# FofanovLab/mtsv_tools

Hardware: AMD Instinct MI355X
Metric: reads/sec (whole node), 150bp reads vs MG-index (higher is better)
Workload: dtype u32/i16

## Files before the change

mtsv_tools_amd/csrc/batch.hip:

```cpp
#include <atomic>
#include <chrono>
#include <cmath>
#include <condition_variable>
#include <exception>
#include <mutex>
#include <thread>
#include <cstdio>
#include <cstdlib>
#include <cstring>
#include <stdexcept>
#include <vector>

#include "../../include/mtsv_amd.h"
#include "batch.hpp"
#include "kernels.hpp"

namespace mtsv {

namespace {
template <class F>
void parallel_ranges(uint64_t n, F f) {
    static const int max_nt = [] {
        const char* e = getenv("MTSV_COPY_THREADS");
        return e ? std::max(1, std::min(16, atoi(e))) : 4;
// ... 209 lines not shown
    sw_ms_acc = 0;
    sweep_ms_acc = diag_ms_acc = bound_ms_acc = edit_ms_acc = 0;
    sw_passed_acc = 0;
    n_hits_total = 0;
    HIP_CHECK(hipMemsetAsync(d_counters, 0, kCounters * sizeof(uint64_t), stream));
    HIP_CHECK(hipEventRecord(ev[8], stream));
}

void Batch::finish_lane() {
    HIP_CHECK(hipEventRecord(ev[9], stream));
    launch_publish(stream, d_counters, h_counters, kCounters);
    HIP_CHECK(hipStreamSynchronize(stream));
    HIP_CHECK(hipEventElapsedTime(&stage_acc[7], ev[8], ev[9]));
    if (getenv("MTSV_TRACE")) fprintf(stderr, "[lane] last pass: %llu strands of 13..64 seed hits (or more than 4 candidates) to k_coalesce_mid, %llu heavier ones\n",
                                      (unsigned long long)(h_counters[15] & 0xffffffffull), (unsigned long long)(h_counters[1] >> 32));
    stats.sw_cell_pairs = h_counters[14];
    stats.sw_prefilter_ms = sw_ms_acc;
    stats.sw_sweep_ms = sweep_ms_acc;
    stats.sw_diag_ms = diag_ms_acc;
    stats.sw_bound_ms = bound_ms_acc;
    stats.edit_ms = edit_ms_acc;
    stats.myers_columns = h_counters[19];
    stats.n_sw_bound_refuted = h_counters[20];
    stats.n_sw_passed = sw_passed_acc + h_counters[21];
    stats.lf_steps = h_counters[2];
    stats.n_candidates = h_counters[3];
    stats.n_verified = h_counters[4];
    stats.window_bytes = h_counters[5];
}

// ... 179 lines not shown
            dev_alloc(&d_seed_pre, want, &dummy);
            seed_cap = want;
        }
        const bool myers_pass = !tiled && pass_max_len <= 253 && (verify_mode == 1 || (sw_pairs && hit_cap < 0x80000000ull));
        const uint32_t plane_words = myers_pass ? myers_words(pass_max_len) : 0;
        if ((uint64_t)nr * 3 * plane_words > plane_cap) {
            (void)hipFree(d_planes);
            d_planes = nullptr;
            const uint64_t want = std::max<uint64_t>(nr, ws_reads) * 3 * plane_words;
            uint64_t dummy = 0;
            dev_alloc(&d_planes, want, &dummy);
            plane_cap = want;
        }
        HIP_CHECK(hipEventRecord(ev[0], stream));
        const uint32_t listed_cap = (uint32_t)std::min<uint64_t>(slots, std::max<uint64_t>(4096, (uint64_t)((double)slots * listed_share)));
        launch_search(stream, v, sb, so, (uint32_t)r0, nr, max_ns, K, G, d_seed_lo, d_seed_cnt, d_seed_pre, (uint32_t*)(d_counters + 22), listed_cap);
        HIP_CHECK(hipEventRecord(ev[1], stream));
        if (max_ns)
            launch_thin(stream, sb, so, (uint32_t)r0, nr, p.edit_rate, p.min_seed, max_ns, K, G, p.max_hits, p.tune_max_hits, d_seed_cnt,
                        d_seed_pre, d_strand_hits, d_strand_nseeds, myers_pass ? d_planes : nullptr, plane_words);
        else {
            HIP_CHECK(hipMemsetAsync(d_strand_hits, 0, (uint64_t)nstr * 4, stream));
            HIP_CHECK(hipMemsetAsync(d_strand_nseeds, 0, (uint64_t)nstr * 4, stream));
        }
        launch_scan(stream, d_strand_hits, nstr, d_tile_sums, d_counters + 0, d_strand_off);
        launch_publish(stream, d_counters, h_counters, 1);
        launch_publish(stream, d_counters + 22, h_counters + 22, 1);
        HIP_CHECK(hipEventRecord(ev[2], stream));
        HIP_CHECK(hipStreamSynchronize(stream));
        {
            const uint64_t n_listed = h_counters[22] & 0xffffffffull;
// ... 792 lines not shown
```

mtsv_tools_amd/csrc/batch.hpp:

```cpp
#pragma once
#include <memory>
#include <mutex>
#include <vector>

#include "../../include/mtsv_amd.h"
#include "host_pack.hpp"
#include "dev_index.hpp"
#include "kernels.hpp"

namespace mtsv {

struct Batch {
    mtsv_index* ix;
    DeviceIndex* di;
    hipStream_t stream = nullptr, copy_stream2 = nullptr;
    mtsv_hit* h_hits_stage = nullptr;
    uint64_t h_hits_cap = 0, staged_hits = 0, last_total_hits = 0;
    bool staged_valid = false;
    struct Arena {
        uint8_t* d_bases = nullptr;
        uint8_t* d_packed = nullptr;
        uint32_t* d_off = nullptr;
        uint64_t cap_bases = 0, cap_reads = 0;
    };
// ... 35 lines not shown
    uint64_t *d_hit_key = nullptr, *d_cand_tmp = nullptr;
    uint4 *d_cand = nullptr, *d_out = nullptr;
    uint32_t *d_cand_next = nullptr, *d_cand_status = nullptr, *d_heavy_list = nullptr;
    DevHit* d_hits = nullptr;
    uint2* d_strip = nullptr;
    uint64_t strip_cap = 0;
    uint32_t* d_planes = nullptr;
    uint64_t plane_cap = 0;
    uint64_t* h_counters = nullptr;
    hipEvent_t ev[15];
    float sw_ms_acc = 0, sweep_ms_acc = 0, diag_ms_acc = 0, bound_ms_acc = 0, edit_ms_acc = 0;
    uint64_t sw_passed_acc = 0;

    std::vector<uint32_t> h_read_off;
    uint32_t max_len = 0;
    static constexpr int kCounters = 24;
    double listed_share = 0.125;
    bool sw_diag = true;
    bool sw_top = true;
    bool sw_bound = true;
    bool sw_fused = true;
    bool sw_prepass = true;
    bool sw_pairs = true;
    int verify_mode = 0;
    uint64_t n_reads = 0;
    uint64_t n_hits_total = 0;
    mtsv_batch_stats stats{};
    float stage_acc[MTSV_N_STAGES] = {0};

    Batch(mtsv_index* ix, DeviceIndex* di, uint64_t max_reads, uint64_t max_bases, uint64_t hit_cap, Batch* parent = nullptr, int lanes = 0);
    ~Batch();
// ... 50 lines not shown
```

mtsv_tools_amd/csrc/dev_index.hip:

```cpp
#include <algorithm>
#include <cstdio>
#include <cstdlib>
#include <cstring>
#include <stdexcept>
#include <thread>
#include <vector>

#include "dev_index.hpp"

namespace mtsv {

void throw_hip(hipError_t e, const char* what, const char* file, int line) {
    throw std::runtime_error(std::string("device: ") + hipGetErrorString(e) + " at " + what + " (" + file + ":" +
                             std::to_string(line) + ")");
}

DeviceIndex::~DeviceIndex() {
    if (device < 0) return;
    (void)hipSetDevice(device);
    (void)hipFree(d_blocks);
    (void)hipFree(d_sa_sample);
    (void)hipFree(d_sa_full);
    (void)hipFree(d_text);
    (void)hipFree(d_bin_end);
    (void)hipFree(d_bins);
    (void)hipFree(d_bin_lut);
    (void)hipFree(d_kmer);
}

namespace {

inline uint32_t sym_code(uint8_t c) {
    switch (c) {
    case 'A': return kCodeA;
    case 'C': return kCodeC;
    case 'G': return kCodeG;
    case 'T': return kCodeT;
    case 'N': return kCodeN;
    case '$': return kCodeSentinel;
    default: return 7;
    }
}
// ... 255 lines not shown
        uint64_t entries = 1ull << (2 * k);
        uint2 *ta = nullptr, *tb = nullptr;
        if (k == 17) {
            if (hipMalloc((void**)&ta, entries * 8) != hipSuccess || hipMalloc((void**)&tb, entries / 4 * 8) != hipSuccess) {
                (void)hipGetLastError();
                if (ta) (void)hipFree(ta);
                ta = tb = nullptr;
                k = 16;
                entries = 1ull << 32;
            }
        }
        if (!ta) {
            HIP_CHECK(hipMalloc((void**)&ta, entries * 8));
            HIP_CHECK(hipMalloc((void**)&tb, std::max<uint64_t>(entries / 4, 4) * 8));
        }
        uint2* cur = (k % 2 == 1) ? ta : tb;
        uint2* oth = (k % 2 == 1) ? tb : ta;
        hipLaunchKernelGGL(k_kmer_level1, dim3(1), dim3(64), 0, 0, v, cur);
        for (uint32_t lvl = 2; lvl <= k; lvl++) {
            const uint64_t total = 1ull << (2 * lvl);
            hipLaunchKernelGGL(k_kmer_level, dim3((uint32_t)std::min<uint64_t>((total + 255) / 256, 1u << 22)), dim3(256), 0, 0, v, cur, oth,
                               2 * (lvl - 1));
            std::swap(cur, oth);
        }
        HIP_CHECK(hipGetLastError());
        HIP_CHECK(hipDeviceSynchronize());
        HIP_CHECK(hipFree(tb));
        di->d_kmer = ta;
        di->bytes += entries * 8;
        v.kmer_tab = di->d_kmer;
        v.kmer_k = k;
        const char* kp = getenv("MTSV_KMER_POS");
        if (v.sa_full && !(kp && atoi(kp) == 0)) {
            unsigned long long* d_n = nullptr;
            HIP_CHECK(hipMalloc((void**)&d_n, sizeof(unsigned long long)));
            HIP_CHECK(hipMemset(d_n, 0, sizeof(unsigned long long)));
            hipEvent_t t0, t1;
            HIP_CHECK(hipEventCreate(&t0));
            HIP_CHECK(hipEventCreate(&t1));
            HIP_CHECK(hipEventRecord(t0, 0));
            hipLaunchKernelGGL(k_kmer_tag, dim3((uint32_t)std::min<uint64_t>((entries + 255) / 256, 1u << 16)), dim3(256), 0, 0, v,
                               di->d_kmer, entries, d_n);
            HIP_CHECK(hipGetLastError());
            HIP_CHECK(hipEventRecord(t1, 0));
            unsigned long long n_tagged = 0;
            HIP_CHECK(hipMemcpy(&n_tagged, d_n, sizeof(n_tagged), hipMemcpyDeviceToHost));
// ... 22 lines not shown
```

mtsv_tools_amd/csrc/dev_index.hpp:

```cpp
#pragma once
#include <map>
#include <memory>
#include <mutex>
#include <string>

#include "dev_layout.hpp"
#include "mgindex.hpp"

namespace mtsv {

[[noreturn]] void throw_hip(hipError_t e, const char* what, const char* file, int line);
#define HIP_CHECK(expr)                                              \
    do {                                                             \
        hipError_t _e = (expr);                                      \
        if (_e != hipSuccess) ::mtsv::throw_hip(_e, #expr, __FILE__, __LINE__); \
    } while (0)

struct DeviceIndex {
    int device = -1;
    RankBlock* d_blocks = nullptr;
    uint32_t* d_sa_sample = nullptr;
    uint32_t* d_sa_full = nullptr;
    uint8_t* d_text = nullptr;
    uint32_t* d_bin_end = nullptr;
    DevBin* d_bins = nullptr;
    uint32_t* d_bin_lut = nullptr;
    uint2* d_kmer = nullptr;
    DevIndexView view{};
    uint64_t bytes = 0;
    uint32_t flags = 0;
    float accel_build_ms = 0.f;

    DeviceIndex() = default;
    DeviceIndex(const DeviceIndex&) = delete;
    DeviceIndex& operator=(const DeviceIndex&) = delete;
    ~DeviceIndex();
};

std::unique_ptr<DeviceIndex> upload_index(const HostIndex& hx, int device, uint32_t flags);

}

// ... 11 lines not shown
```

mtsv_tools_amd/csrc/dev_layout.hpp:

```cpp
#pragma once
#include <hip/hip_runtime.h>

#include <cstdint>

namespace mtsv {

constexpr uint32_t kCodeA = 0, kCodeC = 1, kCodeG = 2, kCodeT = 3, kCodeN = 4, kCodeSentinel = 5;
constexpr uint32_t kBlockRows = 128;
constexpr uint32_t kBlockShift = 7;

struct alignas(64) RankBlock {
    uint32_t cnt[4];
    uint64_t p0[2];
    uint64_t p1[2];
    uint64_t p2[2];
};
static_assert(sizeof(RankBlock) == 64, "rank block must be one 64-byte line");

struct DevBin {
    uint32_t start, end, tax_id, gi;
};

struct DevIndexView {
    const RankBlock* blocks;
// ... 10 lines not shown
    const DevBin* bins;
    uint32_t n_bins;
    const uint32_t* bin_lut;
    uint32_t bin_lut_shift;
    const uint2* kmer_tab;
    uint32_t kmer_k;
};

constexpr uint32_t kKmerTag = 0xFFFFFF00u;
__host__ __device__ inline bool kmer_tagged(uint2 e) { return (e.y & kKmerTag) == kKmerTag; }
__host__ __device__ inline uint32_t kmer_tag_c1(uint2 e) { return e.y & 7u; }
__host__ __device__ inline uint32_t kmer_tag_c2(uint2 e) { return (e.y >> 3) & 7u; }
__host__ __device__ inline uint2 kmer_tag_entry(uint32_t p, uint32_t c1, uint32_t c2) {
    return make_uint2(p, kKmerTag | c1 | (c2 << 3));
}

constexpr uint32_t kSeedAtPos = 0xFFFFFFFFu;

__host__ __device__ inline uint32_t base_code(uint8_t b) {
    switch (b) {
    case 'A': case 'a': return kCodeA;
    case 'C': case 'c': return kCodeC;
    case 'G': case 'g': return kCodeG;
    case 'T': case 't': return kCodeT;
    default: return kCodeN;
    }
}
__host__ __device__ inline uint32_t comp_code(uint32_t c) { return c < 4 ? 3 - c : c; }

#ifdef __HIPCC__
// ... 57 lines not shown
```

mtsv_tools_amd/csrc/k_coalesce.hip:

```cpp
#include "kernels_common.hpp"

namespace mtsv {

namespace {

__device__ inline uint64_t wave_bitonic_sort(uint64_t key) {
    const uint32_t lane = lane_id();
    for (uint32_t k = 2; k <= kWave; k <<= 1)
        for (uint32_t j = k >> 1; j > 0; j >>= 1) {
            uint64_t other = __shfl_xor(key, j);
            bool up = (lane & k) == 0;
            bool lower = (lane & j) == 0;
            key = (lower == up) ? min(key, other) : max(key, other);
        }
    return key;
}

__device__ inline uint32_t find_bin(const DevIndexView& ix, uint32_t site) {
    const uint32_t k = site >> ix.bin_lut_shift;
    uint32_t lo = ix.bin_lut[k], hi = ix.bin_lut[k + 1];
    while (lo < hi) {
        uint32_t mid = (lo + hi) >> 1;
        if (ix.bin_end[mid] <= site)
            lo = mid + 1;
        else
            hi = mid;
    }
    return lo;
}

__device__ inline bool candidate_window(uint32_t site, uint32_t q, const DevBin& bin, uint32_t L, uint32_t ED,
                                        uint32_t* ws, uint32_t* we) {
    uint32_t start_offset = q + ED;
// ... 92 lines not shown
    uint32_t maxc;
    const uint32_t* strand_off;
    const uint32_t* strand_nseeds;
    const uint32_t* hit_ref;
    const uint32_t* hit_q;
    uint64_t* hit_key;
    uint64_t* cand_tmp;
    uint4* cand;
    uint32_t* cand_next;
    uint32_t* cand_status;
    uint32_t* strand_ncand;
    uint32_t* worklist;
    uint32_t* wl_count;
    unsigned long long* n_cand_total;
};

template <bool BLK>
__device__ void coalesce_big(const DevIndexView& ix, const HeavyArgs& a, uint32_t rs, KeyMem<BLK> km, uint32_t* sh_nc) {
    const uint32_t lane = lane_id();
    const uint32_t tid = km.tid(), nt = km.nthreads();
    const bool walker = !BLK || threadIdx.x < kWave;
    const uint32_t o = a.strand_off[rs];
    const uint32_t nh = a.strand_off[rs + 1] - o;
    const uint32_t ns_raw = a.strand_nseeds[rs];
    const bool hopeless = (ns_raw & kHopeless) != 0;
    const StrandGeom g = strand_geom(a.read_off, a.r0 + (rs >> 1), ns_raw);
    for (uint32_t i = tid; i < nh; i += nt) km.st(i, ((uint64_t)a.hit_ref[o + i] << 32) | a.hit_q[o + i]);
    km.sync();
    big_sort(km, nh);
    uint32_t nc = 0;
    uint64_t* ct = a.cand_tmp + 2ull * o;
    if (walker) {
        Walk w{false, 0, 0, 0, 0};
        for (uint32_t base = 0; base < nh; base += kWave) {
            uint32_t cntv = min((uint32_t)kWave, nh - base);
            uint32_t b = 0, ws = 0, we = 0;
            bool ok = false;
            if (lane < cntv) {
                uint64_t key = km.ld(base + lane);
                uint32_t site = (uint32_t)(key >> 32), q = (uint32_t)key;
                b = min(find_bin(ix, site), ix.n_bins - 1);
                DevBin bin = ix.bins[b];
                ok = candidate_window(site, q, bin, g.L, g.ED, &ws, &we);
            }
            for (uint32_t i = 0; i < cntv; i++) {
                uint32_t wsi = __builtin_amdgcn_readlane(ws, i), wei = __builtin_amdgcn_readlane(we, i);
                uint32_t bi = __builtin_amdgcn_readlane(b, i);
                bool oki = __builtin_amdgcn_readlane((uint32_t)ok, i) != 0;
                bool merge = w.have && oki && bi == w.b && ((w.s <= wsi && wsi < w.e) || (w.s < wei && wei <= w.e));
                if (merge) {
                    w.s = min(w.s, wsi);
                    w.e = max(w.e, wei);
                    w.n++;
                } else {
                    if (w.have && w.n >= g.min_seeds) {
                        if (lane == 0) {
                            gstore(ct + 2ull * nc, ((uint64_t)w.e << 32) | w.s);
                            gstore(ct + 2ull * nc + 1, ((uint64_t)w.n << 32) | w.b);
// ... 21 lines not shown
        unsigned long long wsum = 0;
        for (uint32_t i = tid; i < nc; i += nt) {
            const uint64_t se = gload(ct + 2ull * i);
            wsum += (uint32_t)(se >> 32) - (uint32_t)se;
        }
        for (int d = 32; d > 0; d >>= 1) wsum += __shfl_down(wsum, d);
        if (lane == 0 && wsum) atomicAdd(a.n_cand_total + 2, wsum);
        if (tid == 0) {
            a.strand_ncand[rs] = 0;
            if (nc) {
                atomicAdd(a.n_cand_total, (unsigned long long)nc);
                atomicAdd(a.n_cand_total + 1, (unsigned long long)nc);
            }
        }
        km.sync();
        return;
    }
    for (uint32_t i = tid; i < nc; i += nt) {
        uint32_t n_i = (uint32_t)(gload(ct + 2ull * i + 1) >> 32);
        km.st(i, ((uint64_t)(0xffffffffu - n_i) << 32) | i);
    }
    km.sync();
    big_sort(km, nc);
    for (uint32_t base = 0; base < nc; base += nt) {
        uint32_t i = base + tid;
        uint64_t taxkey = 0;
        if (i < nc) {
            uint32_t src = (uint32_t)km.ld(i);
            uint64_t se = gload(ct + 2ull * src), bn = gload(ct + 2ull * src + 1);
            a.cand[o + i] = make_uint4((uint32_t)se, (uint32_t)(se >> 32), (uint32_t)bn, rs);
            a.cand_status[o + i] = 0;
// ... 21 lines not shown
            emit = (p == 0 || (kp >> 32) != (k0 >> 32)) && rk < a.maxc && !hopeless;
        }
        unsigned long long em = __ballot(emit);
        if (em) {
            uint32_t b2 = 0;
            if (lane == 0) b2 = atomicAdd(a.wl_count, (uint32_t)__popcll(em));
            b2 = __builtin_amdgcn_readfirstlane(b2);
            if (emit) a.worklist[b2 + __popcll(em & ((1ull << lane) - 1))] = o + rk;
        }
    }
    if (tid == 0) {
        a.strand_ncand[rs] = hopeless ? 0 : nc;
        if (nc) atomicAdd(a.n_cand_total, (unsigned long long)nc);
    }
    km.sync();
}

template <uint32_t KEYS>
__global__ __launch_bounds__(256) void k_coalesce_heavy(DevIndexView ix, HeavyArgs a, const uint32_t* __restrict__ heavy_list,
                                                        uint32_t list_len, const uint32_t* __restrict__ heavy_count) {
    __shared__ uint64_t lk[KEYS];
    __shared__ uint32_t sh_nc;
    const uint32_t n_heavy = *heavy_count;
    for (uint32_t h = blockIdx.x; h < n_heavy; h += gridDim.x) {
        const uint32_t rs = heavy_list[list_len - 1 - h];
        const uint32_t nh = a.strand_off[rs + 1] - a.strand_off[rs];
        if (KEYS == kHeavyKeysSmall ? nh > kHeavyKeysSmall : nh <= kHeavyKeysSmall) continue;
        if (nh <= KEYS) {
            coalesce_big<true>(ix, a, rs, KeyMem<true>{lk}, &sh_nc);
        } else {
            if (threadIdx.x < kWave) coalesce_big<false>(ix, a, rs, KeyMem<false>{a.hit_key + a.strand_off[rs]}, nullptr);
            __syncthreads();
        }
    }
}


struct CoalesceArgs {
    const uint32_t* read_off;
    uint32_t r0, n_strands;
    uint32_t maxc;
    const uint32_t* strand_off;
    const uint32_t* strand_nseeds;
    const uint32_t* hit_ref;
    const uint32_t* hit_q;
    uint4* cand;
    uint32_t* cand_next;
    uint32_t* cand_status;
// ... 423 lines not shown
    a.maxc = rank_bound(max_candidates);
    a.strand_off = strand_off;
    a.strand_nseeds = strand_nseeds;
    a.hit_ref = hit_ref;
    a.hit_q = hit_q;
    a.hit_key = hit_key;
    a.cand_tmp = cand_tmp;
    a.cand = cand;
    a.cand_next = cand_next;
    a.cand_status = cand_status;
    a.strand_ncand = strand_ncand;
    a.worklist = worklist;
    a.wl_count = wl_count;
    a.n_cand_total = n_cand_total;
    const dim3 hgrid(std::min<uint32_t>(std::max<uint32_t>(n_strands / 64, 1), 2048));
    hipLaunchKernelGGL(k_coalesce_heavy<kHeavyKeysSmall>, hgrid, dim3(256), 0, s, ix, a, heavy_list, n_strands, heavy_count);
    hipLaunchKernelGGL(k_coalesce_heavy<kHeavyKeys>, dim3(std::min<uint32_t>(hgrid.x, 512)), dim3(256), 0, s, ix, a, heavy_list, n_strands, heavy_count);
}

namespace {
__global__ __launch_bounds__(256) void k_max_window(uint32_t n_strands, const uint32_t* __restrict__ strand_off,
                                                    const uint32_t* __restrict__ strand_ncand, const uint4* __restrict__ cand,
                                                    unsigned long long* __restrict__ out) {
    const uint32_t rs = blockIdx.x * blockDim.x + threadIdx.x;
    uint32_t m = 0;
    if (rs < n_strands) {
        const uint32_t o = strand_off[rs], nc = strand_ncand[rs];
        for (uint32_t i = 0; i < nc; i++) {
            const uint4 c = cand[o + i];
            m = max(m, c.y - c.x);
        }
    }
// ... 12 lines not shown
```

mtsv_tools_amd/csrc/k_seed.hip:

```cpp
#include "kernels_common.hpp"

namespace mtsv {

namespace {

__device__ inline uint32_t fast_code(uint32_t ch);
__global__ __launch_bounds__(256) void k_normalise(const uint8_t* src, uint8_t* dst, uint64_t lo, uint64_t hi) {
    const uint64_t i = (lo & ~15ull) + ((uint64_t)blockIdx.x * blockDim.x + threadIdx.x) * 16;
    if (i >= hi) return;
    if (i < lo || i + 16 > hi) {
        const uint64_t a = i < lo ? lo : i, b = i + 16 > hi ? hi : i + 16;
        for (uint64_t q = a; q < b; q++) dst[q] = (uint8_t)fast_code(src[q]);
        return;
    }
    uint4 v = *reinterpret_cast<const uint4*>(src + i);
    uint32_t w[4] = {v.x, v.y, v.z, v.w};
#pragma unroll
    for (int k = 0; k < 4; k++) {
        uint32_t o = 0;
#pragma unroll
        for (int q = 0; q < 4; q++) o |= fast_code((w[k] >> (8 * q)) & 0xffu) << (8 * q);
        w[k] = o;
    }
    *reinterpret_cast<uint4*>(dst + i) = make_uint4(w[0], w[1], w[2], w[3]);
// ... 19 lines not shown
    *reinterpret_cast<uint4*>(dst + i) = make_uint4(w[0], w[1], w[2], w[3]);
}

__device__ inline uint32_t fast_code(uint32_t ch) {
    uint32_t uc = ch & 0xDFu;
    uint32_t x = (uc >> 1) & 3u;
    uint32_t c = x ^ (x >> 1);
    bool acgt = uc == 'A' || uc == 'C' || uc == 'G' || uc == 'T';
    return acgt ? c : kCodeN;
}

constexpr uint32_t kMaxPackedSeed = 32;

__device__ inline void search_slot(const DevIndexView& ix, const uint8_t* __restrict__ bases, const uint32_t* __restrict__ read_off,
                                   uint32_t r0, uint32_t max_ns, uint32_t K, uint32_t G, uint64_t slot,
                                   uint32_t* __restrict__ seed_lo, uint32_t* __restrict__ seed_cnt) {

    uint32_t j = (uint32_t)(slot % max_ns);
    uint64_t rs = slot / max_ns;
    uint32_t strand = (uint32_t)(rs & 1);
    uint32_t r = r0 + (uint32_t)(rs >> 1);
    uint32_t b0 = read_off[r], L = read_off[r + 1] - b0;
    uint32_t ns = n_seeds_of(L, K, G);
    uint32_t lo = 0, hi = 0;
    bool at_pos = false;
    if (j < ns) {
        const uint8_t* read = bases + b0;
        uint32_t off = j * G;
        uint64_t c_lo = 0, c_hi = 0;
        const bool packed = K <= kMaxPackedSeed;
        const uint32_t s0 = b0 + (strand ? L - off - K : off);
// ... 76 lines not shown
            }
            if (acgt) {
                uint2 iv = ix.kmer_tab[idx];
                lo = iv.x;
                hi = iv.y;
                i = (int)K - 1 - (int)ix.kmer_k;
                if (kmer_tagged(iv)) {
                    const uint32_t p = iv.x, m = (uint32_t)(i + 1);
                    bool match = p >= m;
                    for (uint32_t t = 0; match && t < m; t++) match = sym(t) == ix.text[p - m + t];
                    at_pos = match;
                    lo = match ? p - m : 0;
                    hi = 0;
                    i = -1;
                }
            }
        }
        for (; i >= 0 && lo < hi; i--) {
            uint32_t a = sym((uint32_t)i);
            uint32_t bl = lo >> kBlockShift, bh = hi >> kBlockShift;
            LoadedBlock B0 = load_block(ix.blocks, bl);
            uint32_t nlo = less_of(ix, a) + block_rank(B0, a, bl, lo & (kBlockRows - 1), ix.sentinel_row);
            uint32_t nhi;
            if (bh == bl) {
                nhi = less_of(ix, a) + block_rank(B0, a, bh, hi & (kBlockRows - 1), ix.sentinel_row);
            } else {
                LoadedBlock B1 = load_block(ix.blocks, bh);
                nhi = less_of(ix, a) + block_rank(B1, a, bh, hi & (kBlockRows - 1), ix.sentinel_row);
            }
            lo = nlo;
            hi = nhi;
        }
        if (!at_pos && lo >= hi) lo = hi = 0;
    }
    seed_lo[slot] = lo;
    seed_cnt[slot] = at_pos ? kSeedAtPos : hi - lo;
}

__global__ __launch_bounds__(256) void k_search(DevIndexView ix, const uint8_t* __restrict__ bases,
                                                const uint32_t* __restrict__ read_off, uint32_t r0, uint32_t n_reads,
                                                uint32_t max_ns, uint32_t K, uint32_t G,
                                                uint32_t* __restrict__ seed_lo, uint32_t* __restrict__ seed_cnt) {
    uint64_t slot = (uint64_t)blockIdx.x * blockDim.x + threadIdx.x;
    uint64_t total = (uint64_t)n_reads * 2 * max_ns;
    if (slot >= total) return;
    search_slot(ix, bases, read_off, r0, max_ns, K, G, slot, seed_lo, seed_cnt);
}

template <int KK, bool FRONT_TEXT>
__device__ inline bool fast_slot(const DevIndexView& ix, const uint8_t* __restrict__ bases, const uint32_t* __restrict__ read_off,
                                 uint32_t r0, uint32_t total, uint32_t max_ns, uint32_t K, uint32_t G, uint32_t slot,
                                 uint32_t* __restrict__ seed_lo, uint32_t* __restrict__ seed_cnt) {
    const bool in_range = slot < total;
    const uint32_t rs = in_range ? slot / max_ns : 0, j = in_range ? slot - rs * max_ns : 0;
    const uint32_t strand = rs & 1, r = r0 + (rs >> 1);
    const uint32_t b0 = read_off[r], L = read_off[r + 1] - b0;
    const bool live = in_range && j < n_seeds_of(L, K, G);
    uint32_t lo = 0, hi = 0;
    bool slow = false, at_pos = false;
    if (live) {
        const uint32_t off = j * G;
// ... 148 lines not shown
    if (lane < n_slow) tail_q[at + lane] = slow_q[lane];
    __syncthreads();
    const uint32_t nt = tail_n;
    if (nt) {
        __shared__ uint32_t tail_base;
        if (threadIdx.x == 0) tail_base = atomicAdd(slow_count, nt);
        __syncthreads();
        if (threadIdx.x < nt) slow_list[tail_base + threadIdx.x] = tail_q[threadIdx.x];
    }
}

__global__ __launch_bounds__(256) void k_search_listed(DevIndexView ix, const uint8_t* __restrict__ bases,
                                                       const uint32_t* __restrict__ read_off, uint32_t r0, uint32_t max_ns, uint32_t K,
                                                       uint32_t G, const uint32_t* __restrict__ slow_list,
                                                       const uint32_t* __restrict__ slow_count, uint32_t* __restrict__ seed_lo,
                                                       uint32_t* __restrict__ seed_cnt) {
    const uint32_t i = blockIdx.x * blockDim.x + threadIdx.x;
    if (i >= *slow_count) return;
    search_slot(ix, bases, read_off, r0, max_ns, K, G, slow_list[i], seed_lo, seed_cnt);
}


__global__ __launch_bounds__(256) void k_thin(const uint8_t* __restrict__ bases, const uint32_t* __restrict__ read_off,
                                              uint32_t r0, uint32_t n_reads, double edit_rate, double min_seed,
                                              uint32_t max_ns, uint32_t K, uint32_t G, uint64_t max_hits,
                                              uint64_t tune_max_hits, uint32_t* __restrict__ seed_cnt,
                                              uint32_t* __restrict__ seed_pre, uint32_t* __restrict__ strand_hits,
                                              uint32_t* __restrict__ strand_nseeds, uint32_t* __restrict__ planes,
                                              uint32_t plane_words) {
    uint32_t rs = blockIdx.x * blockDim.x + threadIdx.x;
    if (rs >= n_reads * 2) return;
    uint32_t r = r0 + (rs >> 1);
    const uint32_t b0 = read_off[r];
    uint32_t L = read_off[r + 1] - b0;
// ... 290 lines not shown
}

void launch_normalise(hipStream_t s, const uint8_t* src, uint8_t* dst, uint64_t begin, uint64_t end) {
    if (end <= begin) return;
    const uint64_t n = end - (begin & ~15ull);
    hipLaunchKernelGGL(k_normalise, dim3(cdiv((n + 15) / 16, 256)), dim3(256), 0, s, src, dst, begin, end);
}
void launch_unpack(hipStream_t s, const uint8_t* packed, uint8_t* dst, uint64_t lo, uint64_t hi) {
    if (hi <= lo) return;
    const uint64_t groups = ((hi + 15) >> 4) - (lo >> 4);
    hipLaunchKernelGGL(k_unpack, dim3((uint32_t)cdiv(groups, 256)), dim3(256), 0, s, packed, dst, lo, hi);
}

void launch_search(hipStream_t s, const DevIndexView& ix, const uint8_t* bases, const uint32_t* read_off, uint32_t r0,
                   uint32_t n_reads, uint32_t max_ns, uint32_t K, uint32_t G, uint32_t* seed_lo, uint32_t* seed_cnt,
                   uint32_t* slow_list, uint32_t* slow_count, uint32_t listed_cap) {
    (void)hipMemsetAsync(slow_count, 0, sizeof(uint32_t), s);
    uint64_t total = (uint64_t)n_reads * 2 * max_ns;
    if (!total) return;
    const bool fast = ix.kmer_tab && total < 0xffffffffull && K >= 16 && K <= 24 && ix.kmer_k >= 12 && ix.kmer_k <= 17 &&
                      K >= ix.kmer_k && K - std::min<uint32_t>(ix.kmer_k, 16) <= 8 && !getenv("MTSV_SEARCH_GENERIC");
    if (!fast) {
        hipLaunchKernelGGL(k_search, dim3(cdiv(total, 256)), dim3(256), 0, s, ix, bases, read_off, r0, n_reads, max_ns, K, G,
                           seed_lo, seed_cnt);
        return;
    }
    const dim3 grid(std::min<uint32_t>(cdiv(total, 256), 256 * 16));
#define FAST_CASE(KKV)                                                                                                  \
    if (K - KKV > 2)                                                                                                    \
        hipLaunchKernelGGL((k_search_fast<KKV, true>), grid, dim3(256), 0, s, ix, bases, read_off, r0, (uint32_t)total, max_ns, K, G, \
                           seed_lo, seed_cnt, slow_list, slow_count);                                                   \
    else                                                                                                                \
        hipLaunchKernelGGL((k_search_fast<KKV, false>), grid, dim3(256), 0, s, ix, bases, read_off, r0, (uint32_t)total, max_ns, K, G, \
                           seed_lo, seed_cnt, slow_list, slow_count)
    switch (ix.kmer_k) {
    case 12: FAST_CASE(12); break;
    case 13: FAST_CASE(13); break;
    case 14: FAST_CASE(14); break;
    case 15: FAST_CASE(15); break;
    case 17: FAST_CASE(17); break;
    default: FAST_CASE(16); break;
    }
#undef FAST_CASE
    hipLaunchKernelGGL(k_search_listed, dim3(cdiv(std::max<uint32_t>(listed_cap, 1), 256)), dim3(256), 0, s, ix, bases, read_off, r0, max_ns, K, G,
                       slow_list, slow_count, seed_lo, seed_cnt);
}

void launch_thin(hipStream_t s, const uint8_t* bases, const uint32_t* read_off, uint32_t r0, uint32_t n_reads, double edit_rate,
                 double min_seed, uint32_t max_ns, uint32_t K, uint32_t G, uint64_t max_hits, uint64_t tune, uint32_t* seed_cnt, uint32_t* seed_pre,
                 uint32_t* strand_hits, uint32_t* strand_nseeds, uint32_t* planes, uint32_t plane_words) {
    hipLaunchKernelGGL(k_thin, dim3(cdiv((uint64_t)n_reads * 2, 256)), dim3(256), 0, s, bases, read_off, r0, n_reads, edit_rate,
                       min_seed, max_ns, K, G, max_hits, tune, seed_cnt, seed_pre, strand_hits, strand_nseeds, planes, plane_words);
}

void launch_scan(hipStream_t s, const uint32_t* in, uint32_t n, uint64_t* tile_sums, uint64_t* total, uint32_t* out) {
    uint32_t tiles = cdiv(n ? n : 1, kScanTile);
    hipLaunchKernelGGL(k_scan_tile_sums, dim3(tiles), dim3(kScanThreads), 0, s, in, n, tile_sums);
    hipLaunchKernelGGL(k_scan_sums, dim3(1), dim3(1024), 0, s, tile_sums, tiles, total);
    hipLaunchKernelGGL(k_scan_apply, dim3(tiles), dim3(kScanThreads), 0, s, in, n, tile_sums, total, out);
}
// ... 21 lines not shown
```

mtsv_tools_amd/csrc/kernels.hpp:

```cpp
#pragma once
#include <algorithm>

#include "dev_layout.hpp"

namespace mtsv {

struct DevHit {
    uint64_t read;
    uint32_t tax_id;
    uint32_t gi;
    uint32_t edit;
    uint8_t strand;
    uint8_t pad[3];
    uint64_t offset;
};
static_assert(sizeof(DevHit) == 32, "DevHit must match mtsv_hit");

constexpr uint32_t kCtrVerified = 4, kCtrWindowBytes = 5, kCtrSwCursor = 8, kCtrPassCount = 9, kCtrSwCellPairs = 14;

struct EvalArgs {
    const uint8_t* bases;
    const uint32_t* read_off;
    uint32_t r0;
    double edit_rate;
    int64_t max_candidates;
    const uint32_t* strand_off;
    const uint4* cand;
    const uint32_t* cand_next;
    uint32_t* cand_status;
    const uint32_t* worklist;
    const uint32_t* wl_count;
    uint32_t* wl_cursor;
    uint32_t wl_reverse = 0;
// ... 16 lines not shown
    uint32_t plane_words = 0;
    uint32_t maxc = 0xffffffffu;
    uint32_t claim_shift = 0;
};

inline uint32_t myers_words(uint32_t max_len) { return std::min(std::max((max_len + 31) / 32, 2u), 8u); }

constexpr uint32_t kMaxRegisterReadLen = 256;
constexpr uint32_t kMaxReadLen = 32767;

void launch_publish(hipStream_t s, const uint64_t* src, uint64_t* dst_host, uint32_t n);
void launch_normalise(hipStream_t s, const uint8_t* src, uint8_t* dst, uint64_t begin, uint64_t end);
void launch_unpack(hipStream_t s, const uint8_t* packed, uint8_t* dst, uint64_t lo, uint64_t hi);
void launch_search(hipStream_t s, const DevIndexView& ix, const uint8_t* bases, const uint32_t* read_off, uint32_t r0,
                   uint32_t n_reads, uint32_t max_ns, uint32_t K, uint32_t G, uint32_t* seed_lo, uint32_t* seed_cnt,
                   uint32_t* slow_list, uint32_t* slow_count, uint32_t listed_cap);
void launch_thin(hipStream_t s, const uint8_t* bases, const uint32_t* read_off, uint32_t r0, uint32_t n_reads, double edit_rate,
                 double min_seed, uint32_t max_ns, uint32_t K, uint32_t G, uint64_t max_hits, uint64_t tune, uint32_t* seed_cnt, uint32_t* seed_pre,
                 uint32_t* strand_hits, uint32_t* strand_nseeds, uint32_t* planes, uint32_t plane_words);
void launch_scan(hipStream_t s, const uint32_t* in, uint32_t n, uint64_t* tile_sums, uint64_t* total, uint32_t* out);
uint32_t scan_tiles(uint32_t n);
void launch_expand(hipStream_t s, const DevIndexView& ix, uint32_t n_strands, uint32_t max_ns, uint32_t G,
                   const uint32_t* seed_lo, const uint32_t* seed_cnt, const uint32_t* seed_pre, const uint32_t* strand_off,
                   uint32_t* hit_row, uint32_t* hit_ref, uint32_t* hit_q);
void launch_locate(hipStream_t s, const DevIndexView& ix, uint32_t total_hits_host, const uint32_t* total_hits_dev,
                   const uint32_t* hit_row, uint32_t* hit_ref, unsigned long long* lf_steps);
void launch_coalesce(hipStream_t s, const DevIndexView& ix, const uint32_t* read_off, uint32_t r0, uint32_t n_strands,
                     int64_t max_candidates, const uint32_t* strand_off,
                     const uint32_t* strand_nseeds, const uint32_t* hit_ref, const uint32_t* hit_q, uint64_t* hit_key,
                     uint64_t* cand_tmp, uint4* cand, uint32_t* cand_next, uint32_t* cand_status,
                     uint32_t* strand_ncand, uint32_t* worklist, uint32_t* heavy_list, uint64_t* counters);
// ... 19 lines not shown
```

Before: 396.5 million.

## Parallelize heavy-strand coalescing by bin runs and keep k-mer prefix levels for seeding

The heavy coalesce kernel for strands with up to the small key count now computes candidate windows for all hits across the whole block and merges each run of equal bins in parallel, one thread per run start. A block prefix sum then compacts the kept candidates, and blocks pull strands through an atomic ticket counter instead of a fixed stride. If any run exceeds a length cap, the kernel falls back to the serial wavefront walk, reusing the windows it already computed. Separately, the index builder keeps every intermediate k-mer table level up to 12, so the generic and listed seed-search paths can start backward search from a short-prefix interval when the full k-mer lookup does not apply. This costs extra device memory and shared memory, which may lower occupancy of the heavy kernel.

After: 413.5 million, median of 6. 1.04x the previous value.

```diff
diff --git a/mtsv_tools_amd/csrc/batch.hip b/mtsv_tools_amd/csrc/batch.hip
--- a/mtsv_tools_amd/csrc/batch.hip
+++ b/mtsv_tools_amd/csrc/batch.hip
@@ -247,6 +247,8 @@
     HIP_CHECK(hipEventElapsedTime(&stage_acc[7], ev[8], ev[9]));
     if (getenv("MTSV_TRACE")) fprintf(stderr, "[lane] last pass: %llu strands of 13..64 seed hits (or more than 4 candidates) to k_coalesce_mid, %llu heavier ones\n",
                                       (unsigned long long)(h_counters[15] & 0xffffffffull), (unsigned long long)(h_counters[1] >> 32));
+    if (getenv("MTSV_TRACE")) fprintf(stderr, "[lane] k_coalesce_heavy: %llu strands walked by runs, %llu by the wavefront walk (a run too long)\n",
+                                      (unsigned long long)(h_counters[kCtrHeavyWalk] & 0xffffffffull), (unsigned long long)(h_counters[kCtrHeavyWalk] >> 32));
     stats.sw_cell_pairs = h_counters[14];
     stats.sw_prefilter_ms = sw_ms_acc;
     stats.sw_sweep_ms = sweep_ms_acc;
@@ -456,7 +458,7 @@
         }
         HIP_CHECK(hipEventRecord(ev[0], stream));
         const uint32_t listed_cap = (uint32_t)std::min<uint64_t>(slots, std::max<uint64_t>(4096, (uint64_t)((double)slots * listed_share)));
-        launch_search(stream, v, sb, so, (uint32_t)r0, nr, max_ns, K, G, d_seed_lo, d_seed_cnt, d_seed_pre, (uint32_t*)(d_counters + 22), listed_cap);
+        launch_search(stream, v, sb, so, (uint32_t)r0, nr, max_ns, K, G, d_seed_lo, d_seed_cnt, d_seed_pre, (uint32_t*)(d_counters + 22), listed_cap, di->d_kmer_levels);
         HIP_CHECK(hipEventRecord(ev[1], stream));
         if (max_ns)
             launch_thin(stream, sb, so, (uint32_t)r0, nr, p.edit_rate, p.min_seed, max_ns, K, G, p.max_hits, p.tune_max_hits, d_seed_cnt,
diff --git a/mtsv_tools_amd/csrc/batch.hpp b/mtsv_tools_amd/csrc/batch.hpp
--- a/mtsv_tools_amd/csrc/batch.hpp
+++ b/mtsv_tools_amd/csrc/batch.hpp
@@ -73,7 +73,7 @@
 
     std::vector<uint32_t> h_read_off;
     uint32_t max_len = 0;
-    static constexpr int kCounters = 24;
+    static constexpr int kCounters = 25;
     double listed_share = 0.125;
     bool sw_diag = true;
     bool sw_top = true;
diff --git a/mtsv_tools_amd/csrc/dev_index.hip b/mtsv_tools_amd/csrc/dev_index.hip
--- a/mtsv_tools_amd/csrc/dev_index.hip
+++ b/mtsv_tools_amd/csrc/dev_index.hip
@@ -26,6 +26,7 @@
     (void)hipFree(d_bins);
     (void)hipFree(d_bin_lut);
     (void)hipFree(d_kmer);
+    (void)hipFree(d_kmer_levels);
 }
 
 namespace {
@@ -311,14 +312,29 @@
             HIP_CHECK(hipMalloc((void**)&ta, entries * 8));
             HIP_CHECK(hipMalloc((void**)&tb, std::max<uint64_t>(entries / 4, 4) * 8));
         }
+        const char* kl = getenv("MTSV_KMER_LEVELS");
+        const uint32_t n_levels = ((kl && atoi(kl) == 0) || !v.sa_full) ? 0 : std::min(k, kKmerLevelsMax);
+        uint64_t level_bytes = 0;
+        if (n_levels) {
+            level_bytes = (uint64_t)kmer_level_start(n_levels + 1) * sizeof(uint2);
+            HIP_CHECK(hipMalloc((void**)&di->d_kmer_levels, level_bytes));
+            di->bytes += level_bytes;
+        }
+        auto keep_level = [&](uint32_t lvl, const uint2* src) {
+            if (lvl <= n_levels)
+                HIP_CHECK(hipMemcpyAsync(di->d_kmer_levels + kmer_level_start(lvl), src, (sizeof(uint2)) << (2 * lvl),
+                                         hipMemcpyDeviceToDevice, 0));
+        };
         uint2* cur = (k % 2 == 1) ? ta : tb;
         uint2* oth = (k % 2 == 1) ? tb : ta;
         hipLaunchKernelGGL(k_kmer_level1, dim3(1), dim3(64), 0, 0, v, cur);
+        keep_level(1, cur);
         for (uint32_t lvl = 2; lvl <= k; lvl++) {
             const uint64_t total = 1ull << (2 * lvl);
             hipLaunchKernelGGL(k_kmer_level, dim3((uint32_t)std::min<uint64_t>((total + 255) / 256, 1u << 22)), dim3(256), 0, 0, v, cur, oth,
                                2 * (lvl - 1));
             std::swap(cur, oth);
+            keep_level(lvl, cur);
         }
         HIP_CHECK(hipGetLastError());
         HIP_CHECK(hipDeviceSynchronize());
@@ -327,6 +343,8 @@
         di->bytes += entries * 8;
         v.kmer_tab = di->d_kmer;
         v.kmer_k = k;
+        if (getenv("MTSV_TRACE"))
+            fprintf(stderr, "[upload] kmer levels 1..%u kept: %llu bytes\n", n_levels, (unsigned long long)level_bytes);
         const char* kp = getenv("MTSV_KMER_POS");
         if (v.sa_full && !(kp && atoi(kp) == 0)) {
             unsigned long long* d_n = nullptr;
diff --git a/mtsv_tools_amd/csrc/dev_index.hpp b/mtsv_tools_amd/csrc/dev_index.hpp
--- a/mtsv_tools_amd/csrc/dev_index.hpp
+++ b/mtsv_tools_amd/csrc/dev_index.hpp
@@ -26,6 +26,7 @@
     DevBin* d_bins = nullptr;
     uint32_t* d_bin_lut = nullptr;
     uint2* d_kmer = nullptr;
+    uint2* d_kmer_levels = nullptr;
     DevIndexView view{};
     uint64_t bytes = 0;
     uint32_t flags = 0;
diff --git a/mtsv_tools_amd/csrc/dev_layout.hpp b/mtsv_tools_amd/csrc/dev_layout.hpp
--- a/mtsv_tools_amd/csrc/dev_layout.hpp
+++ b/mtsv_tools_amd/csrc/dev_layout.hpp
@@ -48,6 +48,9 @@
 __host__ __device__ inline uint2 kmer_tag_entry(uint32_t p, uint32_t c1, uint32_t c2) {
     return make_uint2(p, kKmerTag | c1 | (c2 << 3));
 }
+
+constexpr uint32_t kKmerLevelsMax = 12;
+__host__ __device__ inline uint32_t kmer_level_start(uint32_t j) { return ((1u << (2 * j)) - 4u) / 3u; }
 
 constexpr uint32_t kSeedAtPos = 0xFFFFFFFFu;
 
diff --git a/mtsv_tools_amd/csrc/k_coalesce.hip b/mtsv_tools_amd/csrc/k_coalesce.hip
--- a/mtsv_tools_amd/csrc/k_coalesce.hip
+++ b/mtsv_tools_amd/csrc/k_coalesce.hip
@@ -1,3 +1,5 @@
+#include <cstring>
+
 #include "kernels_common.hpp"
 
 namespace mtsv {
@@ -16,7 +18,8 @@
     return key;
 }
 
-__device__ inline uint32_t find_bin(const DevIndexView& ix, uint32_t site) {
+template <class V>
+__device__ inline uint32_t find_bin(const V& ix, uint32_t site) {
     const uint32_t k = site >> ix.bin_lut_shift;
     uint32_t lo = ix.bin_lut[k], hi = ix.bin_lut[k + 1];
     while (lo < hi) {
@@ -139,9 +142,115 @@
     uint32_t* wl_count;
     unsigned long long* n_cand_total;
 };
+__device__ inline uint32_t* heavy_counter(const HeavyArgs& a, uint32_t slot) {
+    return reinterpret_cast<uint32_t*>(a.n_cand_total + slot - 3);
+}
+
+constexpr uint32_t kRunMax = 256;
+struct RunMem {
+    uint32_t bin[kHeavyKeysSmall];
+    uint32_t kept[kHeavyKeysSmall / 32];
+    uint32_t too_long;
+    uint32_t wave_sum[256 / kWave];
+};
+static_assert(kHeavyKeysSmall == 256 * 8, "walk_by_runs: eight hits per thread in the compaction");
+struct BinView {
+    const uint32_t* bin_end;
+    const DevBin* bins;
+    uint32_t n_bins;
+    const uint32_t* bin_lut;
+    uint32_t bin_lut_shift;
+};
+
+constexpr uint32_t kRunTooLong = 0xffffffffu;
+__device__ __attribute__((noinline)) uint32_t walk_by_runs(BinView ix, StrandGeom g, uint64_t* keys, RunMem& rm, uint32_t nh, uint64_t* ct) {
+    const uint32_t tid = threadIdx.x;
+    for (uint32_t i = tid; i < nh; i += 256) {
+        const uint64_t key = keys[i];
+        const uint32_t site = (uint32_t)(key >> 32), q = (uint32_t)key;
+        const uint32_t b = min(find_bin(ix, site), ix.n_bins - 1);
+        const DevBin bin = ix.bins[b];
+        uint32_t ws, we;
+        const bool ok = candidate_window(site, q, bin, g.L, g.ED, &ws, &we);
+        keys[i] = ((uint64_t)we << 32) | ws;
+        rm.bin[i] = b | (ok ? 0x80000000u : 0u);
+    }
+    if (tid < kHeavyKeysSmall / 32) rm.kept[tid] = 0;
+    if (tid == 0) rm.too_long = 0;
+    __syncthreads();
+    for (uint32_t h = tid; h < nh; h += 256) {
+        const uint32_t v = rm.bin[h];
+        if (!(v >> 31)) continue;
+        if (h && rm.bin[h - 1] == v) continue;
+        const uint32_t b = v & 0x7fffffffu;
+        const uint64_t se = keys[h];
+        uint32_t s = (uint32_t)se, e = (uint32_t)(se >> 32), n = 1;
+        auto keep = [&](uint32_t last) {
+            if (n >= g.min_seeds) {
+                gstore(ct + 2ull * last, ((uint64_t)e << 32) | s);
+                gstore(ct + 2ull * last + 1, ((uint64_t)n << 32) | b);
+                atomicOr(&rm.kept[last >> 5], 1u << (last & 31));
+            }
+        };
+        uint32_t j = h + 1;
+        for (; j < nh && rm.bin[j] == v; j++) {
+            if (j - h >= kRunMax) {
+                rm.too_long = 1;
+                break;
+            }
+            const uint64_t x = keys[j];
+            const uint32_t wsj = (uint32_t)x, wej = (uint32_t)(x >> 32);
+            if ((s <= wsj && wsj < e) || (s < wej && wej <= e)) {
+                s = min(s, wsj);
+                e = max(e, wej);
+                n++;
+            } else {
+                keep(j - 1);
+                s = wsj; e = wej; n = 1;
+            }
+        }
+        keep(j - 1);
+    }
+    wave_mem_sync();
+    __syncthreads();
+    if (rm.too_long) return kRunTooLong;
+    const uint32_t bits = (rm.kept[tid >> 2] >> (8 * (tid & 3))) & 0xffu;
+    const uint32_t cnt = __popc(bits);
+    uint32_t incl = cnt;
+    for (int d = 1; d < kWave; d <<= 1) {
+        const uint32_t up = (uint32_t)__shfl_up((int)incl, d);
+        if (lane_id() >= (uint32_t)d) incl += up;
+    }
+    if (lane_id() == kWave - 1) rm.wave_sum[tid / kWave] = incl;
+    uint64_t r0[8], r1[8];
+#pragma unroll
+    for (int k = 0; k < 8; k++) {
+        r0[k] = r1[k] = 0;
+        if (bits >> k & 1) {
+            r0[k] = gload(ct + 2ull * (8 * tid + k));
+            r1[k] = gload(ct + 2ull * (8 * tid + k) + 1);
+        }
+    }
+    __syncthreads();
+    uint32_t pos = incl - cnt, total = 0;
+#pragma unroll
+    for (uint32_t w = 0; w < 256 / kWave; w++) {
+        if (w < tid / kWave) pos += rm.wave_sum[w];
+        total += rm.wave_sum[w];
+    }
+#pragma unroll
+    for (int k = 0; k < 8; k++)
+        if (bits >> k & 1) {
+            gstore(ct + 2ull * pos, r0[k]);
+            gstore(ct + 2ull * pos + 1, r1[k]);
+            pos++;
+        }
+    return total;
+}
 
 template <bool BLK>
-__device__ void coalesce_big(const DevIndexView& ix, const HeavyArgs& a, uint32_t rs, KeyMem<BLK> km, uint32_t* sh_nc) {
+__device__ bool coalesce_big(const DevIndexView& ix, const HeavyArgs& a, uint32_t rs, KeyMem<BLK> km, uint32_t* sh_nc,
+                             RunMem* rm = nullptr) {
     const uint32_t lane = lane_id();
     const uint32_t tid = km.tid(), nt = km.nthreads();
     const bool walker = !BLK || threadIdx.x < kWave;
@@ -155,7 +264,15 @@
     big_sort(km, nh);
     uint32_t nc = 0;
     uint64_t* ct = a.cand_tmp + 2ull * o;
-    if (walker) {
+    bool by_runs = false, pre = false;
+    if (BLK && rm) {
+        nc = walk_by_runs(BinView{ix.bin_end, ix.bins, ix.n_bins, ix.bin_lut, ix.bin_lut_shift}, g, km.p, *rm, nh, ct);
+        by_runs = nc != kRunTooLong;
+        pre = !by_runs;
+        if (!by_runs) nc = 0;
+        else if (threadIdx.x == 0) *sh_nc = nc;
+    }
+    if (walker && !by_runs) {
         Walk w{false, 0, 0, 0, 0};
         for (uint32_t base = 0; base < nh; base += kWave) {
             uint32_t cntv = min((uint32_t)kWave, nh - base);
@@ -163,10 +280,17 @@
             bool ok = false;
             if (lane < cntv) {
                 uint64_t key = km.ld(base + lane);
-                uint32_t site = (uint32_t)(key >> 32), q = (uint32_t)key;
-                b = min(find_bin(ix, site), ix.n_bins - 1);
-                DevBin bin = ix.bins[b];
-                ok = candidate_window(site, q, bin, g.L, g.ED, &ws, &we);
+                if (pre) {
+                    ws = (uint32_t)key;
+                    we = (uint32_t)(key >> 32);
+                    b = rm->bin[base + lane] & 0x7fffffffu;
+                    ok = (rm->bin[base + lane] >> 31) != 0;
+                } else {
+                    uint32_t site = (uint32_t)(key >> 32), q = (uint32_t)key;
+                    b = min(find_bin(ix, site), ix.n_bins - 1);
+                    DevBin bin = ix.bins[b];
+                    ok = candidate_window(site, q, bin, g.L, g.ED, &ws, &we);
+                }
             }
             for (uint32_t i = 0; i < cntv; i++) {
                 uint32_t wsi = __builtin_amdgcn_readlane(ws, i), wei = __builtin_amdgcn_readlane(we, i);
@@ -218,7 +342,7 @@
             }
         }
         km.sync();
-        return;
+        return by_runs;
     }
     for (uint32_t i = tid; i < nc; i += nt) {
         uint32_t n_i = (uint32_t)(gload(ct + 2ull * i + 1) >> 32);
@@ -270,24 +394,51 @@
         if (nc) atomicAdd(a.n_cand_total, (unsigned long long)nc);
     }
     km.sync();
-}
-
-template <uint32_t KEYS>
+    return by_runs;
+}
+
+template <uint32_t KEYS, bool RUNS>
 __global__ __launch_bounds__(256) void k_coalesce_heavy(DevIndexView ix, HeavyArgs a, const uint32_t* __restrict__ heavy_list,
                                                         uint32_t list_len, const uint32_t* __restrict__ heavy_count) {
+    static_assert(!RUNS || KEYS == kHeavyKeysSmall, "the walk by runs is sized for the small key array");
     __shared__ uint64_t lk[KEYS];
     __shared__ uint32_t sh_nc;
+    __shared__ RunMem rm;
+    __shared__ uint32_t sh_ticket;
     const uint32_t n_heavy = *heavy_count;
-    for (uint32_t h = blockIdx.x; h < n_heavy; h += gridDim.x) {
+    uint32_t n_walked = 0;
+    uint32_t h = blockIdx.x;
+    for (;;) {
+        if (RUNS) {
+            if (threadIdx.x == 0) sh_ticket = atomicAdd(heavy_counter(a, kCtrHeavyTicket), 1u);
+            __syncthreads();
+            h = sh_ticket;
+        }
+        if (h >= n_heavy) break;
         const uint32_t rs = heavy_list[list_len - 1 - h];
         const uint32_t nh = a.strand_off[rs + 1] - a.strand_off[rs];
-        if (KEYS == kHeavyKeysSmall ? nh > kHeavyKeysSmall : nh <= kHeavyKeysSmall) continue;
-        if (nh <= KEYS) {
-            coalesce_big<true>(ix, a, rs, KeyMem<true>{lk}, &sh_nc);
-        } else {
-            if (threadIdx.x < kWave) coalesce_big<false>(ix, a, rs, KeyMem<false>{a.hit_key + a.strand_off[rs]}, nullptr);
-            __syncthreads();
-        }
+        const bool other = KEYS == kHeavyKeysSmall ? nh > kHeavyKeysSmall : nh <= kHeavyKeysSmall;
+        if (!other) {
+            if (nh <= KEYS) {
+                if (RUNS) {
+                    const bool by_runs = coalesce_big<true>(ix, a, rs, KeyMem<true>{lk}, &sh_nc, &rm);
+                    asm volatile("" : "+v"(n_walked));
+                    n_walked += by_runs ? 1u : 0x10000u;
+                } else {
+                    coalesce_big<true>(ix, a, rs, KeyMem<true>{lk}, &sh_nc);
+                }
+            } else {
+                if (threadIdx.x < kWave) coalesce_big<false>(ix, a, rs, KeyMem<false>{a.hit_key + a.strand_off[rs]}, nullptr);
+                __syncthreads();
+            }
+        }
+        if (RUNS) __syncthreads();
+        else h += gridDim.x;
+    }
+    if (RUNS && threadIdx.x == 0) {
+        uint32_t* c = heavy_counter(a, kCtrHeavyWalk);
+        if (n_walked & 0xffffu) atomicAdd(c, n_walked & 0xffffu);
+        if (n_walked >> 16) atomicAdd(c + 1, n_walked >> 16);
     }
 }
 
@@ -741,8 +892,15 @@
     a.wl_count = wl_count;
     a.n_cand_total = n_cand_total;
     const dim3 hgrid(std::min<uint32_t>(std::max<uint32_t>(n_strands / 64, 1), 2048));
-    hipLaunchKernelGGL(k_coalesce_heavy<kHeavyKeysSmall>, hgrid, dim3(256), 0, s, ix, a, heavy_list, n_strands, heavy_count);
-    hipLaunchKernelGGL(k_coalesce_heavy<kHeavyKeys>, dim3(std::min<uint32_t>(hgrid.x, 512)), dim3(256), 0, s, ix, a, heavy_list, n_strands, heavy_count);
+    const char* hw = getenv("MTSV_HEAVY_WALK");
+    const bool serial_walk = hw && !strcmp(hw, "serial");
+    if (serial_walk || ix.n_bins >= 0x80000000u) {
+        hipLaunchKernelGGL((k_coalesce_heavy<kHeavyKeysSmall, false>), hgrid, dim3(256), 0, s, ix, a, heavy_list, n_strands, heavy_count);
+    } else {
+        (void)hipMemsetAsync(counters + kCtrHeavyTicket, 0, sizeof(uint64_t), s);
+        hipLaunchKernelGGL((k_coalesce_heavy<kHeavyKeysSmall, true>), hgrid, dim3(256), 0, s, ix, a, heavy_list, n_strands, heavy_count);
+    }
+    hipLaunchKernelGGL((k_coalesce_heavy<kHeavyKeys, false>), dim3(std::min<uint32_t>(hgrid.x, 512)), dim3(256), 0, s, ix, a, heavy_list, n_strands, heavy_count);
 }
 
 namespace {
diff --git a/mtsv_tools_amd/csrc/k_seed.hip b/mtsv_tools_amd/csrc/k_seed.hip
--- a/mtsv_tools_amd/csrc/k_seed.hip
+++ b/mtsv_tools_amd/csrc/k_seed.hip
@@ -57,7 +57,8 @@
 
 __device__ inline void search_slot(const DevIndexView& ix, const uint8_t* __restrict__ bases, const uint32_t* __restrict__ read_off,
                                    uint32_t r0, uint32_t max_ns, uint32_t K, uint32_t G, uint64_t slot,
-                                   uint32_t* __restrict__ seed_lo, uint32_t* __restrict__ seed_cnt) {
+                                   uint32_t* __restrict__ seed_lo, uint32_t* __restrict__ seed_cnt,
+                                   const uint2* __restrict__ levels) {
 
     uint32_t j = (uint32_t)(slot % max_ns);
     uint64_t rs = slot / max_ns;
@@ -164,6 +165,20 @@
                     hi = 0;
                     i = -1;
                 }
+            } else if (levels) {
+                const uint32_t Lk = min(ix.kmer_k, kKmerLevelsMax);
+                uint32_t m = 0, lidx = 0;
+                for (; m < Lk; m++) {
+                    const uint32_t a = sym(K - 1 - m);
+                    if (a > 3) break;
+                    lidx |= a << (2 * m);
+                }
+                if (m) {
+                    const uint2 iv = levels[kmer_level_start(m) + lidx];
+                    lo = iv.x;
+                    hi = iv.y;
+                    i = (int)K - 1 - (int)m;
+                }
             }
         }
         for (; i >= 0 && lo < hi; i--) {
@@ -190,11 +205,12 @@
 __global__ __launch_bounds__(256) void k_search(DevIndexView ix, const uint8_t* __restrict__ bases,
                                                 const uint32_t* __restrict__ read_off, uint32_t r0, uint32_t n_reads,
                                                 uint32_t max_ns, uint32_t K, uint32_t G,
-                                                uint32_t* __restrict__ seed_lo, uint32_t* __restrict__ seed_cnt) {
+                                                uint32_t* __restrict__ seed_lo, uint32_t* __restrict__ seed_cnt,
+                                                const uint2* __restrict__ levels) {
     uint64_t slot = (uint64_t)blockIdx.x * blockDim.x + threadIdx.x;
     uint64_t total = (uint64_t)n_reads * 2 * max_ns;
     if (slot >= total) return;
-    search_slot(ix, bases, read_off, r0, max_ns, K, G, slot, seed_lo, seed_cnt);
+    search_slot(ix, bases, read_off, r0, max_ns, K, G, slot, seed_lo, seed_cnt, levels);
 }
 
 template <int KK, bool FRONT_TEXT>
@@ -373,10 +389,10 @@
                                                        const uint32_t* __restrict__ read_off, uint32_t r0, uint32_t max_ns, uint32_t K,
                                                        uint32_t G, const uint32_t* __restrict__ slow_list,
                                                        const uint32_t* __restrict__ slow_count, uint32_t* __restrict__ seed_lo,
-                                                       uint32_t* __restrict__ seed_cnt) {
+                                                       uint32_t* __restrict__ seed_cnt, const uint2* __restrict__ levels) {
     const uint32_t i = blockIdx.x * blockDim.x + threadIdx.x;
     if (i >= *slow_count) return;
-    search_slot(ix, bases, read_off, r0, max_ns, K, G, slow_list[i], seed_lo, seed_cnt);
+    search_slot(ix, bases, read_off, r0, max_ns, K, G, slow_list[i], seed_lo, seed_cnt, levels);
 }
 
 
@@ -697,7 +713,7 @@
 
 void launch_search(hipStream_t s, const DevIndexView& ix, const uint8_t* bases, const uint32_t* read_off, uint32_t r0,
                    uint32_t n_reads, uint32_t max_ns, uint32_t K, uint32_t G, uint32_t* seed_lo, uint32_t* seed_cnt,
-                   uint32_t* slow_list, uint32_t* slow_count, uint32_t listed_cap) {
+                   uint32_t* slow_list, uint32_t* slow_count, uint32_t listed_cap, const uint2* kmer_levels) {
     (void)hipMemsetAsync(slow_count, 0, sizeof(uint32_t), s);
     uint64_t total = (uint64_t)n_reads * 2 * max_ns;
     if (!total) return;
@@ -705,7 +721,7 @@
                       K >= ix.kmer_k && K - std::min<uint32_t>(ix.kmer_k, 16) <= 8 && !getenv("MTSV_SEARCH_GENERIC");
     if (!fast) {
         hipLaunchKernelGGL(k_search, dim3(cdiv(total, 256)), dim3(256), 0, s, ix, bases, read_off, r0, n_reads, max_ns, K, G,
-                           seed_lo, seed_cnt);
+                           seed_lo, seed_cnt, kmer_levels);
         return;
     }
     const dim3 grid(std::min<uint32_t>(cdiv(total, 256), 256 * 16));
@@ -726,7 +742,7 @@
     }
 #undef FAST_CASE
     hipLaunchKernelGGL(k_search_listed, dim3(cdiv(std::max<uint32_t>(listed_cap, 1), 256)), dim3(256), 0, s, ix, bases, read_off, r0, max_ns, K, G,
-                       slow_list, slow_count, seed_lo, seed_cnt);
+                       slow_list, slow_count, seed_lo, seed_cnt, kmer_levels);
 }
 
 void launch_thin(hipStream_t s, const uint8_t* bases, const uint32_t* read_off, uint32_t r0, uint32_t n_reads, double edit_rate,
diff --git a/mtsv_tools_amd/csrc/kernels.hpp b/mtsv_tools_amd/csrc/kernels.hpp
--- a/mtsv_tools_amd/csrc/kernels.hpp
+++ b/mtsv_tools_amd/csrc/kernels.hpp
@@ -17,6 +17,7 @@
 static_assert(sizeof(DevHit) == 32, "DevHit must match mtsv_hit");
 
 constexpr uint32_t kCtrVerified = 4, kCtrWindowBytes = 5, kCtrSwCursor = 8, kCtrPassCount = 9, kCtrSwCellPairs = 14;
+constexpr uint32_t kCtrHeavyWalk = 23, kCtrHeavyTicket = 24;
 
 struct EvalArgs {
     const uint8_t* bases;
@@ -63,7 +64,7 @@
 void launch_unpack(hipStream_t s, const uint8_t* packed, uint8_t* dst, uint64_t lo, uint64_t hi);
 void launch_search(hipStream_t s, const DevIndexView& ix, const uint8_t* bases, const uint32_t* read_off, uint32_t r0,
                    uint32_t n_reads, uint32_t max_ns, uint32_t K, uint32_t G, uint32_t* seed_lo, uint32_t* seed_cnt,
-                   uint32_t* slow_list, uint32_t* slow_count, uint32_t listed_cap);
+                   uint32_t* slow_list, uint32_t* slow_count, uint32_t listed_cap, const uint2* kmer_levels);
 void launch_thin(hipStream_t s, const uint8_t* bases, const uint32_t* read_off, uint32_t r0, uint32_t n_reads, double edit_rate,
                  double min_seed, uint32_t max_ns, uint32_t K, uint32_t G, uint64_t max_hits, uint64_t tune, uint32_t* seed_cnt, uint32_t* seed_pre,
                  uint32_t* strand_hits, uint32_t* strand_nseeds, uint32_t* planes, uint32_t plane_words);
```
